# MasterVVK/qwen3-tts-axera-russian

Hardware: AMD Instinct MI355X
Metric: 12Hz codec-tokens/s (codec frames/s, 16 codes each) + RTF, Qwen3-TTS-0.6B (higher is better)
Workload: dtype f16 weights/KV, f32 accumulate (talker+CP); vocoder exact fp32 (f32 MFMA); 1 GPU; configs[2]/[3]: batch=32 mixed ru/en prompts per GPU, 64 frames/utterance/step (prefill + hipGraph decode loop), utterance-sharded DP over 1 GPU(s); batch_per_gpu=32

## Files before the change

include/qwen3tts_voc.h:

```cpp
#ifndef QWEN3TTS_VOC_H
#define QWEN3TTS_VOC_H

#include <stdint.h>

#ifdef __cplusplus
extern "C" {
#endif

#define Q3VOC_SAMPLES_PER_TOKEN 1920
#define Q3VOC_SAMPLE_RATE 24000

void* voc_load(const char* weights, int chunk_tokens, int max_batch);
void voc_free(void* v);
int voc_chunk_tokens(void* v);
int voc_samples_per_token(void* v);
int voc_chunk_samples(void* v);

int voc_decode(void* v, const int64_t* codes, int B, float* out);

int voc_synthesize(void* v, const int64_t* codes, int n_tokens, int16_t* out, int32_t* n_samples);
int voc_synthesize_f32(void* v, const int64_t* codes, int n_tokens, float* out, int32_t* n_samples);
int voc_synthesize_max_samples(void* v, int n_tokens);

int voc_synthesize_batch(void* v, const int64_t* codes, const int32_t* n_tokens, int U, int16_t* out, int64_t out_capacity,
// ... 16 lines not shown
int voc_stream_last_chunks(void* s);
float voc_stream_last_ms(void* s);

void* voc_incr_create(void* voc, int max_streams);
void voc_incr_free(void* s);
int voc_incr_reset(void* s, int stream);
int64_t voc_incr_push_max_samples(void* s, int n, const int32_t* streams, const int32_t* n_new, const int32_t* finish);
int voc_incr_push(void* s, int n, const int32_t* streams, const int64_t* codes, const int32_t* n_new, const int32_t* finish,
                  int16_t* out, int64_t out_capacity, int64_t* offsets);
int voc_incr_push_f32(void* s, int n, const int32_t* streams, const int64_t* codes, const int32_t* n_new, const int32_t* finish,
                      float* out, int64_t out_capacity, int64_t* offsets);
float voc_incr_last_ms(void* s);
int voc_incr_last_launches(void* s);
int64_t voc_incr_samples(void* voc, int64_t n_frames);
int64_t voc_incr_state_bytes(void* s);
int64_t voc_incr_device_bytes(void* s);

int voc_set_exact_fp32(int on);

int voc_set_fused_units(int on);

int voc_set_max_workgroups(int n);

float voc_last_decode_ms(void* v);
double voc_decode_flops(void* v, int B);

#ifdef __cplusplus
}
#endif
#endif
```

qwen3_tts_axera_russian_amd/csrc/q3_test_api.hip:

```cpp
#include "q3_model.h"
#include "q3_voc_ops.h"
#include <chrono>
#include <cstring>
#include <vector>

using namespace q3;

namespace q3 {
int set_linear_tuning(int K, int mt16, int kbw);
int set_linear_split_rows(int on);
int set_linear_narrow8(int on);
int set_linear_wide_tiles(int on);
int set_attn_short(int on);
int set_gemm_min_rows(int n);
int set_gemm_glds(int on);
int reset_linear_knobs();
const char* last_linear_variant();
}

namespace {
struct DBuf {
    void* p = nullptr;
    ~DBuf() {
        if (p) hipFree(p);
// ... 328 lines not shown
}

int q3t_voc_attn(int kernel, const float* x, float* y, int B, int H, int D, int L, int window, float theta) {
    constexpr float GUARD = 1234.5f;
    if ((kernel != 0 && kernel != 1) || !x || !y || B <= 0 || H <= 0 || D <= 0 || D > 128 || (D & 1) || L <= 0 || window <= 0)
        return -2;
    const int ld = (L + 31) / 32 * 32;
    const size_t nx = (size_t)B * 3 * H * D, ny = (size_t)B * H * D;
    std::vector<float> hx(nx * ld, 0.f), hy(ny * ld, GUARD);
    for (size_t r = 0; r < nx; r++) memcpy(hx.data() + r * ld, x + r * L, (size_t)L * 4);
    DBuf dx, dy;
    if (!dx.up(hx.data(), hx.size() * 4) || !dy.up(hy.data(), hy.size() * 4)) return -1;
    const int rc = kernel == 0 ? voc_launch_attn(nullptr, (const float*)dx.p, (float*)dy.p, H, D, L, ld, window, theta, B)
                               : voc_launch_attn_tile(nullptr, (const float*)dx.p, (float*)dy.p, H, D, L, ld, window, theta, B);
    if (rc) return -2;
    Q3_HIP(hipDeviceSynchronize(), -1);
    Q3_HIP(hipMemcpy(hy.data(), dy.p, hy.size() * 4, hipMemcpyDeviceToHost), -1);
    for (size_t r = 0; r < ny; r++) {
        memcpy(y + r * L, hy.data() + r * ld, (size_t)L * 4);
        for (int l = L; l < ld; l++)
            if (hy[r * ld + l] != GUARD) return -3;
    }
    return 0;
}

float q3t_bench_linear(int M, int N, int K, int pro, int epi, int nt, int n_copies, int iters) {
    hipStream_t s = nullptr;
    if (hipStreamCreate(&s) != hipSuccess) return -1.f;
    const size_t wbytes = (size_t)N * K * 2;
    const int Mreal = M;
    M = (M + 127) / 128 * 128;
    DBuf dW, dx, dh, dssq, dg, dy, dso, dact;
    if (!dW.alloc(wbytes * n_copies)) return -1.f;
    hipMemset(dW.p, 0x11, wbytes * n_copies);
    dx.alloc((size_t)M * K * 2);
    hipMemset(dx.p, 0, (size_t)M * K * 2);
    dh.alloc((size_t)M * K * 4);
    hipMemset(dh.p, 0, (size_t)M * K * 4);
    dssq.alloc((size_t)M * (K / 16) * 4);
    hipMemset(dssq.p, 0, (size_t)M * (K / 16) * 4);
    dg.alloc((size_t)K * 4);
    hipMemset(dg.p, 0, (size_t)K * 4);
    dy.alloc((size_t)M * N * 4);
    dso.alloc((size_t)M * (N / 16) * 4);
    dact.alloc((size_t)M * (N / 2) * 2);
    LinArgs a;
// ... 150 lines not shown
```

qwen3_tts_axera_russian_amd/csrc/q3_voc.hip:

```cpp
#include "../../include/qwen3tts_voc.h"
#include "q3_common.h"
#include "q3_voc_ops.h"

#include <algorithm>
#include <cmath>
#include <utility>

namespace q3 {

typedef float f16v __attribute__((ext_vector_type(16)));

enum { VOP_RVQ = 1, VOP_CONV = 2, VOP_CONVT = 3, VOP_DWCONV = 4, VOP_NORM = 5, VOP_ATTN = 6, VOP_GLU = 7, VOP_EMBMEAN = 8 };
enum { VF_SNAKE = 1, VF_RES_ADD = 2, VF_RES_SAVE = 4, VF_CLAMP = 8, VF_GELU = 16 };

__device__ __forceinline__ float gelu_erf(float x) { return 0.5f * x * (1.0f + erff(x * 0.70710678118654752f)); }
__device__ __forceinline__ float elu1(float x) { return x > 0.f ? x : expm1f(x); }


static int g_voc_split = 1;
static int g_voc_max_wgs = 0;
constexpr int VKC = 8;
constexpr int VTN = 128;
#ifndef Q3_VOC_XPAD
#define Q3_VOC_XPAD 1
#endif
#ifndef Q3_VOC_WPAD
#define Q3_VOC_WPAD 0
#endif
__host__ __device__ constexpr int voc_wpitch(int TM) { return Q3_VOC_WPAD ? (TM % 64 == 0 ? TM + 32 : (TM % 64 == 32 ? TM : TM + 4)) : TM + 4; }
__host__ __device__ inline int voc_xpitch(int XW) { return Q3_VOC_XPAD ? ((XW + 31) / 64) * 64 + 32 : XW; }

template <int MT, int KT, int KC, bool CT = false, int ACT = 3>
__global__ void __launch_bounds__(256, (KC >= 32 && MT >= 3) ? 2 : (MT >= 4 ? 3 : (MT == 3 ? 3 : 4))) conv_kernel(ConvArgs a) {
    constexpr int TM = 32 * MT, TMP = voc_wpitch(TM), Q = KC / 4;
    const int tid = threadIdx.x, lane = tid & 63, w = tid >> 6;
    const int halo = (KT - 1) * a.dil;
    const int HA = (halo + 3) & ~3;
    const int XW = VTN + HA;
    const int XP = voc_xpitch(XW);
    extern __shared__ __attribute__((aligned(16))) float lds[];
    float* Ws = lds;
    float* Xs = lds + KT * KC * TMP;
    for (int tile = blockIdx.x; tile < a.n_tiles; tile += gridDim.x) {
        const int lx = tile % a.tiles_l, my = (tile / a.tiles_l) % a.tiles_m, b = tile / (a.tiles_l * a.tiles_m);
        const int l0 = lx * VTN, m0 = my * TM;
        const float* xb = a.x + (size_t)b * a.Cin * a.ldx;
        const int Lcols = a.flat_B > 0 ? a.flat_B * a.ldx : a.Lc;
        f16v acc[MT];
#pragma unroll
        for (int mt = 0; mt < MT; mt++)
#pragma unroll
            for (int i = 0; i < 16; i++) acc[mt][i] = 0.f;
        constexpr int WN = KT * KC * (TM / 4), WIT = (WN + 255) / 256;
        constexpr int LPC = 256 / KC;
        constexpr int XJ1 = (VTN / 4 + LPC - 1) / LPC;
        const int xci = tid / LPC, xl = tid - xci * LPC;
        float4 wv[WIT];
        float4 xv1[KT == 1 ? XJ1 : 1];
        float al = 0.f, ib = 0.f;
        auto load_w = [&](int ci0) {
#pragma unroll
            for (int i = 0; i < WIT; i++) {
                const int idx = tid + i * 256, ic = idx < WN ? idx : 0;
                const int m4 = ic % (TM / 4), ci = (ic / (TM / 4)) % KC, k = ic / ((TM / 4) * KC);
                const int m = m0 + m4 * 4, mc = m < a.Mp ? m : 0, cg = ci0 + ci;
                wv[i] = *(const float4*)(a.wk + (unsigned)((((cg >> 3) * KT + k) * 8 + (cg & 7)) * a.Mp + mc));
// ... 146 lines not shown
                    }
                }
            }
        } else if (gl < Lcols) {
#pragma unroll
            for (int mt = 0; mt < MT; mt++)
#pragma unroll
                for (int r = 0; r < 16; r++) {
                    const int m = m0 + mt * 32 + (r & 3) + 8 * (r >> 2) + 4 * (lane >> 5);
                    if (m < a.M) {
                        const int co = a.stride == 1 ? m : m / a.stride;
                        const int p = a.stride == 1 ? 0 : m % a.stride;
                        const int jo = l * a.stride + p - a.lt;
                        if (a.stride != 1 && (jo < 0 || jo >= a.Lout)) continue;
                        const unsigned idx = (unsigned)((be * a.Cout + co) * a.ldy + jo);
                        float v = acc[mt][r];
                        if (a.bias) v += a.bias[co];
                        if (a.res) v += a.res[idx];
                        if (a.clamp) v = fminf(fmaxf(v, -1.f), 1.f);
                        __builtin_nontemporal_store(v, &a.y[idx]);
                    }
                }
        }
    }
}

template <int MT, int KT, int KC, bool CT = false, int ACT = -1>
static int launch_conv_t(hipStream_t s, const ConvArgs& a, int B) {
    if constexpr (!CT && KT <= 2) {
        if (a.stride > 1 && a.res == nullptr) return launch_conv_t<MT, KT, KC, true, ACT>(s, a, B);
    }
    if constexpr (ACT < 0) {
        if (a.elu) {
            if constexpr (!CT && KC == 16 && (KT == 1 || KT == 3)) return launch_conv_t<MT, KT, KC, CT, 4>(s, a, B);
            Q3_LOG("voc conv: ELU input is built for 1- and 3-tap convs at 16 channels per stage only");
            return -1;
        }
        if (a.alpha && a.gelu) {
            Q3_LOG("voc conv: Snake and GELU on one input are not built");
            return -1;
        }
        if constexpr (!(KT == 1 && KC == 16 && MT == 4 && !CT)) return launch_conv_t<MT, KT, KC, CT, 3>(s, a, B);
        else return a.alpha ? launch_conv_t<MT, KT, KC, CT, 1>(s, a, B) : a.gelu ? launch_conv_t<MT, KT, KC, CT, 2>(s, a, B)
                                                                             : launch_conv_t<MT, KT, KC, CT, 0>(s, a, B);
    } else {
    constexpr int TM = 32 * MT, TMP = voc_wpitch(TM);
    const int halo = (KT - 1) * a.dil;
// ... 8 lines not shown
        lds = lds_pad;
        static bool attr = false;
        if (!attr) {
            Q3_HIP(hipFuncSetAttribute((const void*)conv_kernel<MT, KT, KC, CT, ACT>, hipFuncAttributeMaxDynamicSharedMemorySize, 160 * 1024), -1);
            attr = true;
        }
    }
    ConvArgs c = a;
    c.Mp = (a.M + 3) / 4 * 4;
    c.flat_B = (KT == 1 && a.stride == 1) ? B : 0;
    if ((a.ldx & 3) || (a.ldy & 3) || a.ldx < a.Lin || a.ldy < a.Lout || a.Lc < a.Lin || a.Lc > a.Lin + KT - 1) {
        Q3_LOG("voc conv: bad geometry (Lin %d pitch %d, Lout %d pitch %d, Lc %d)", a.Lin, a.ldx, a.Lout, a.ldy, a.Lc);
        return -1;
    }
    {
        if ((size_t)B * a.Cin * a.ldx >= ((size_t)1 << 31) || (size_t)B * a.Cout * a.ldy >= ((size_t)1 << 31)) {
            Q3_LOG("voc conv: activation of %d x %d x %d / %d x %d x %d floats is beyond the kernel's 32-bit indexing", B, a.Cin, a.ldx, B, a.Cout, a.ldy);
            return -1;
        }
    }
    c.tiles_l = ((c.flat_B > 0 ? a.ldx * B : a.Lc) + VTN - 1) / VTN;
    c.tiles_m = (a.M + TM - 1) / TM;
    c.n_tiles = c.tiles_l * c.tiles_m * (c.flat_B > 0 ? 1 : B);
    int grid = c.n_tiles;
    if (g_voc_max_wgs > 0 && grid > g_voc_max_wgs) grid = g_voc_max_wgs;
    hipLaunchKernelGGL((conv_kernel<MT, KT, KC, CT, ACT>), dim3(grid), dim3(256), lds, s, c);
    Q3_HIP(hipGetLastError(), -1);
    return 0;
    }
}

template <int KT, int KC>
static int launch_conv_mt(hipStream_t s, const ConvArgs& a, int B) {
    const int t32 = (a.M + 31) / 32;
    int mt = 4;
    if (t32 % 4 != 0) mt = (t32 % 3 == 0) ? 3 : (t32 % 2 == 0) ? 2 : (t32 < 4 ? t32 : 4);
    static const int fill = getenv("Q3_VOC_FILL") ? atoi(getenv("Q3_VOC_FILL")) : 512;
    if (fill > 0) {
        const long cols = (KT == 1 && a.stride == 1) ? (long)a.ldx * B : (long)a.Lc;
        const long col_tiles = (cols + VTN - 1) / VTN * ((KT == 1 && a.stride == 1) ? 1 : B);
        while (mt > 1 && col_tiles * ((t32 + mt - 1) / mt) < fill) mt = (mt == 4 || mt == 2) ? mt / 2 : 1;
    }
    switch (mt) {
        case 1: return launch_conv_t<1, KT, KC>(s, a, B);
        case 2: return launch_conv_t<2, KT, KC>(s, a, B);
        case 3: return launch_conv_t<3, KT, KC>(s, a, B);
        default: return launch_conv_t<4, KT, KC>(s, a, B);
    }
// ... 77 lines not shown
        return a.K == 1 ? launch_conv_mt<1, 16>(s, a, B) : launch_conv_mt<2, 16>(s, a, B);
    switch (a.K) {
        case 1: return c % 32 == 0 ? launch_conv_mt<1, 32>(s, a, B) : c % 16 == 0 ? launch_conv_mt<1, 16>(s, a, B) : launch_conv_mt<1, 8>(s, a, B);
        case 2: return c % 32 == 0 ? launch_conv_mt<2, 32>(s, a, B) : c % 16 == 0 ? launch_conv_mt<2, 16>(s, a, B) : launch_conv_mt<2, 8>(s, a, B);
        case 3: return c % 16 == 0 ? launch_conv_mt<3, 16>(s, a, B) : launch_conv_mt<3, 8>(s, a, B);
        case 7: return launch_conv_mt<7, 8>(s, a, B);
        default:
            Q3_LOG("voc conv: kernel with %d taps is not built (1, 2, 3, 7 are)", a.K);
            return -1;
    }
}

int voc_launch_conv(hipStream_t s, const ConvArgs& a, int B) { return launch_conv(s, a, B); }

struct ResUnitArgs {
    const float* x = nullptr;
    float* y = nullptr;
    const float* w7 = nullptr;
    const float* w1p = nullptr;
    const float *b7 = nullptr, *b1 = nullptr;
    const float *al7 = nullptr, *ib7 = nullptr;
    const float *al1 = nullptr, *ib1 = nullptr;
    int Lin = 0, ld = 0, dil = 1, tiles_l = 0, n_tiles = 0;
};

static int g_voc_fuse = 1;

template <int MT>
__global__ void __launch_bounds__(256, MT <= 3 ? 3 : 2) resunit_kernel(ResUnitArgs a) {
    constexpr int C = 32 * MT, KT = 7, KC = 8, TMP = voc_wpitch(C);
    const int tid = threadIdx.x, lane = tid & 63, w = tid >> 6;
    const int halo = (KT - 1) * a.dil, HA = (halo + 3) & ~3, XW = VTN + HA, XP = voc_xpitch(XW);
    extern __shared__ __attribute__((aligned(16))) float lds[];
    float* Ws = lds;
    float* Xs = lds + KT * KC * TMP;
    float* Ps = Xs + KC * XP;
    for (int i = tid; i < C; i += 256) {
        Ps[i] = a.b7 ? a.b7[i] : 0.f;
        Ps[C + i] = a.al1[i];
        Ps[2 * C + i] = a.ib1[i];
        Ps[3 * C + i] = a.b1 ? a.b1[i] : 0.f;
    }
    for (int tile = blockIdx.x; tile < a.n_tiles; tile += gridDim.x) {
        const int lx = tile % a.tiles_l, b = tile / a.tiles_l;
        const int l0 = lx * VTN;
        const float* xb = a.x + (size_t)b * C * a.ld;
        f16v acc[MT];
#pragma unroll
        for (int mt = 0; mt < MT; mt++)
#pragma unroll
            for (int i = 0; i < 16; i++) acc[mt][i] = 0.f;
        for (int ci0 = 0; ci0 < C; ci0 += KC) {
            __syncthreads();
            constexpr int WN = KT * KC * (C / 4), WIT = (WN + 255) / 256;
            float4 wv[WIT];
#pragma unroll
            for (int i = 0; i < WIT; i++) {
                const int idx = tid + i * 256, ic = idx < WN ? idx : 0;
                const int m4 = ic % (C / 4), ci = (ic / (C / 4)) % KC, k = ic / ((C / 4) * KC);
                const int cg = ci0 + ci;
                wv[i] = *(const float4*)(a.w7 + (unsigned)((((cg >> 3) * KT + k) * 8 + (cg & 7)) * C + m4 * 4));
            }
            constexpr int LPC = 256 / KC, XG = (VTN + (((KT - 1) * 9 + 3) & ~3)) / 4, XJ = (XG + LPC - 1) / LPC;
            const int xci = tid / LPC, xl = tid - xci * LPC;
            const float al = a.al7[ci0 + xci], ib = a.ib7[ci0 + xci];
            float4 xv[XJ];
// ... 71 lines not shown
            for (int i = 0; i < MT; i++) {
                const int idx = tid + i * 256;
                *(float4*)(Ws + idx * 4) = *(const float4*)(a.w1p + (unsigned)(mt2 * 32 * C + idx * 4));
            }
            __syncthreads();
            f16v o;
#pragma unroll
            for (int i = 0; i < 16; i++) o[i] = 0.f;
#pragma unroll
            for (int mt = 0; mt < MT; mt++)
#pragma unroll
                for (int q = 0; q < 16; q++)
                    o = __builtin_amdgcn_mfma_f32_32x32x2f32(Ws[(mt * 16 + q) * 64 + lane], acc[mt][q], o, 0, 0, 0);
            if (live) {
                float* yb = a.y + (size_t)b * C * a.ld;
#pragma unroll
                for (int r = 0; r < 16; r++) {
                    const int mu = 32 * mt2 + (r & 3) + 8 * (r >> 2);
                    float* rowp = yb + (unsigned)(mu * a.ld);
                    __builtin_nontemporal_store(o[r] + Ps[3 * C + mu + 4 * (lane >> 5)] + res[r], &rowp[lane_off]);
                }
            }
        }
    }
}

template <int MT>
static int launch_resunit_t(hipStream_t s, ResUnitArgs a, int B) {
    constexpr int C = 32 * MT;
    const int halo = 6 * a.dil;
    if (a.dil > 9) return -1;
    const size_t lds = ((size_t)7 * 8 * voc_wpitch(C) + (size_t)8 * voc_xpitch(VTN + ((halo + 3) & ~3)) + 4 * C) * sizeof(float);
    a.tiles_l = (a.Lin + VTN - 1) / VTN;
    a.n_tiles = a.tiles_l * B;
    int grid = a.n_tiles;
    if (g_voc_max_wgs > 0 && grid > g_voc_max_wgs) grid = g_voc_max_wgs;
    hipLaunchKernelGGL((resunit_kernel<MT>), dim3(grid), dim3(256), lds, s, a);
    Q3_HIP(hipGetLastError(), -1);
    return 0;
}

static bool resunit_channels(int c) { return c == 96 || c == 192; }

static int launch_resunit(hipStream_t s, const ResUnitArgs& a, int C, int B) {
    return C == 96 ? launch_resunit_t<3>(s, a, B) : C == 192 ? launch_resunit_t<6>(s, a, B) : -1;
}

typedef _Float16 hv8 __attribute__((ext_vector_type(8)));

__global__ void __launch_bounds__(256) snake_split_kernel(const float* __restrict__ x, const float* __restrict__ alpha,
                                                          const float* __restrict__ inv_beta, _Float16* __restrict__ xh,
                                                          _Float16* __restrict__ xl, int C, int L, int ld, int gelu,
                                                          int* __restrict__ ovf) {
    const int l = blockIdx.x * 256 + threadIdx.x, cg = blockIdx.y, b = blockIdx.z;
    if (l >= L) return;
    const float* xp = x + ((size_t)b * C + cg * 8) * ld + l;
    float v[8];
#pragma unroll
    for (int j = 0; j < 8; j++) v[j] = xp[(size_t)j * ld];
// ... 20 lines not shown
    const size_t o = (((size_t)b * (C >> 3) + cg) * L + l) * 8;
    *(hv8*)(xh + o) = h;
    *(hv8*)(xl + o) = lo;
    if (big) *ovf = 1;
}

struct SplitArgs {
    const _Float16* xh = nullptr;
    const _Float16* xl = nullptr;
    float* y = nullptr;
    const _Float16* w_hi = nullptr;
    const _Float16* w_lo = nullptr;
    const float* bias = nullptr;
    const float* res = nullptr;
    _Float16* oh = nullptr;
    _Float16* ol = nullptr;
    const float* oalpha = nullptr;
    const float* oinv_beta = nullptr;
    int* ovf = nullptr;
    int Cin = 0, M = 0, Mp = 0, dil = 1, Lin = 0, stride = 1, Cout = 0, clamp = 0, B = 0;
    int ldy = 0, lt = 0, Lout = 0, Lc = 0;
    int n_tiles = 0, tiles_l = 0, tiles_m = 0;
    int my_fast = 0;
};

constexpr int SKC = 16;

template <int KT, int KS, int MW, int NJ>
__global__ void __launch_bounds__(256, NJ == 1 ? 3 : 2) conv_split_kernel(SplitArgs a) {
    constexpr int STM = 32 * MW, STN = 128 * NJ;
    constexpr int UNR = (MW == 3 && KT == 7) ? 1 : KS * KT;
    const int tid = threadIdx.x, lane = tid & 63, w = tid >> 6;
    const int halo = (KT - 1) * a.dil;
    const int XW = STN + halo;
    extern __shared__ __attribute__((aligned(16))) char slds[];
    _Float16* Wh = (_Float16*)slds;
    _Float16* Wl = Wh + KS * KT * STM * SKC;
    _Float16* Xh = Wl + KS * KT * STM * SKC;
    _Float16* Xl = Xh + (size_t)KS * XW * SKC;
    const int C16 = a.Cin >> 4;
    const hv8 zero8 = {0, 0, 0, 0, 0, 0, 0, 0};
    for (int tile = blockIdx.x; tile < a.n_tiles; tile += gridDim.x) {
        int lx, b, my;
        if (a.my_fast) {
            const int xcd = tile & 7, j = tile >> 3;
            my = j % a.tiles_m;
            const int cg = (j / a.tiles_m) * 8 + xcd;
            if (cg >= a.tiles_l * a.B) continue;
            lx = cg % a.tiles_l;
            b = cg / a.tiles_l;
        } else {
            lx = tile % a.tiles_l;
            b = (tile / a.tiles_l) % a.B;
            my = tile / (a.tiles_l * a.B);
        }
        const int l0 = lx * STN, m0 = my * STM;
        f16v acc[MW][NJ], accx[MW][NJ];
#pragma unroll
        for (int i = 0; i < MW; i++)
#pragma unroll
            for (int j = 0; j < NJ; j++)
#pragma unroll
                for (int r = 0; r < 16; r++) {
                    acc[i][j][r] = 0.f;
                    accx[i][j][r] = 0.f;
// ... 86 lines not shown
                        if (a.oh && mg < a.M) {
                            hv4 vh, vl;
                            bool big = false;
#pragma unroll
                            for (int q = 0; q < 4; q++) {
                                float t = v[q];
                                if (a.oalpha) {
                                    const float sn = __sinf(a.oalpha[mg + q] * t);
                                    t = t + a.oinv_beta[mg + q] * (sn * sn);
                                }
                                big |= !(fabsf(t) <= 65504.f);
                                const _Float16 hi = (_Float16)fminf(fmaxf(t, -65504.f), 65504.f);
                                vh[q] = hi;
                                vl[q] = (_Float16)((t - (float)hi) * 2048.0f);
                            }
                            if (big) *a.ovf = 1;
                            const size_t o = (((size_t)b * (a.Cout >> 3) + (mg >> 3)) * a.Lin + l) * 8 + (mg & 7);
                            *(hv4*)(a.oh + o) = vh;
                            *(hv4*)(a.ol + o) = vl;
                        }
                    }
                }
            }
    }
}

template <int KT, int KS, int MW, int NJ>
static int launch_conv_split_t(hipStream_t s, const SplitArgs& a, int B) {
    constexpr int STM = 32 * MW, STN = 128 * NJ;
    if (a.dil > 9) return -1;
    const int halo = (KT - 1) * a.dil;
    const size_t lds = ((size_t)2 * KS * KT * STM * SKC + (size_t)2 * KS * (STN + halo) * SKC) * sizeof(_Float16);
    static bool set_ = false;
    if (!set_) {
        Q3_HIP(hipFuncSetAttribute((const void*)conv_split_kernel<KT, KS, MW, NJ>, hipFuncAttributeMaxDynamicSharedMemorySize, 80 * 1024), -1);
        set_ = true;
    }
    if (lds > 80 * 1024 || (a.Cin / 16) % KS || a.Mp % STM) return -1;
    SplitArgs c = a;
    c.B = B;
    c.tiles_l = (a.Lc + STN - 1) / STN;
    c.tiles_m = (a.M + STM - 1) / STM;
    c.n_tiles = c.tiles_l * c.tiles_m * B;
    c.my_fast = c.tiles_m > 1 && (size_t)a.Cin * a.Mp * KT * 4 <= (size_t)2 << 20;
    if (c.my_fast) c.n_tiles = (c.tiles_l * B + 7) / 8 * 8 * c.tiles_m;
    int grid = c.n_tiles;
    if (g_voc_max_wgs > 0 && grid > g_voc_max_wgs) grid = g_voc_max_wgs;
    hipLaunchKernelGGL((conv_split_kernel<KT, KS, MW, NJ>), dim3(grid), dim3(256), lds, s, c);
    Q3_HIP(hipGetLastError(), -1);
    return 0;
}

static int g_voc_narrow_k1 = 1;

template <int MW>
static int launch_conv_split_m(hipStream_t s, const SplitArgs& a, int K, int B) {
    const int c16 = a.Cin / 16;
    switch (K) {
        case 1:
            if (g_voc_narrow_k1 && MW == 3)
                return c16 % 3 == 0 ? launch_conv_split_t<1, 3, MW, 1>(s, a, B) : c16 % 2 == 0 ? launch_conv_split_t<1, 2, MW, 1>(s, a, B) : launch_conv_split_t<1, 1, MW, 1>(s, a, B);
            return c16 % 3 == 0 ? launch_conv_split_t<1, 3, MW, 2>(s, a, B) : c16 % 2 == 0 ? launch_conv_split_t<1, 2, MW, 2>(s, a, B) : launch_conv_split_t<1, 1, MW, 2>(s, a, B);
        case 2:
            if (g_voc_narrow_k1 && MW == 3 && a.Cin <= 384)
                return c16 % 2 == 0 ? launch_conv_split_t<2, 2, MW, 1>(s, a, B) : launch_conv_split_t<2, 1, MW, 1>(s, a, B);
            return c16 % 2 == 0 ? launch_conv_split_t<2, 2, MW, 2>(s, a, B) : launch_conv_split_t<2, 1, MW, 2>(s, a, B);
        case 3: return c16 % 2 == 0 && MW == 2 ? launch_conv_split_t<3, 2, MW, 2>(s, a, B) : launch_conv_split_t<3, 1, MW, 2>(s, a, B);
        case 7:
            if (g_voc_narrow_k1 && a.Cin <= 192) return launch_conv_split_t<7, 1, MW, 1>(s, a, B);
            return launch_conv_split_t<7, 1, MW, 2>(s, a, B);
// ... 426 lines not shown

struct Voc {
    int device = 0;
    int chunk = 64, max_batch = 1, upsample = 1;
    long chunk_samples = 0;
    std::vector<VocOp> ops;
    std::vector<void*> allocs;
    hipStream_t s = nullptr;
    hipEvent_t e0 = nullptr, e1 = nullptr;
    int64_t* d_codes = nullptr;
    int* d_ovf = nullptr;
    bool warned_ovf = false;
    float *buf[3] = {nullptr, nullptr, nullptr};
    _Float16 *plane[4] = {nullptr, nullptr, nullptr, nullptr};
    size_t buf_elems = 0;
    float last_ms = 0.f;
    double flops_per_chunk = 0.0;
    float* d_wave = nullptr;
    int16_t* d_wave16 = nullptr;
    size_t wave_cap = 0, wave16_cap = 0;
    ChunkPlace* d_place = nullptr;
    float batch_ms = 0.f;
    int batch_chunks = 0;
};

static float* voc_up(Voc* v, const PackTensor* t) {
    size_t ne = t->numel();
    std::vector<float> tmp;
    const float* src = (const float*)t->data;
    if (t->dtype == F16) {
        tmp.resize(ne);
        for (size_t i = 0; i < ne; i++) tmp[i] = h2f(((const uint16_t*)t->data)[i]);
        src = tmp.data();
    } else if (t->dtype != F32) {
        return nullptr;
    }
    float* d = nullptr;
    if (hipMalloc((void**)&d, ne * 4) != hipSuccess) return nullptr;
    v->allocs.push_back(d);
    if (hipMemcpy(d, src, ne * 4, hipMemcpyHostToDevice) != hipSuccess) return nullptr;
    return d;
}

static float* voc_up_host(Voc* v, const std::vector<float>& h) {
    float* d = nullptr;
    if (hipMalloc((void**)&d, h.size() * 4) != hipSuccess) return nullptr;
    v->allocs.push_back(d);
    if (hipMemcpy(d, h.data(), h.size() * 4, hipMemcpyHostToDevice) != hipSuccess) return nullptr;
    return d;
}

static void voc_destroy(Voc* v) {
    if (!v) return;
    if (v->s) hipStreamSynchronize(v->s);
    for (void* p : v->allocs) hipFree(p);
    for (float* b : v->buf)
        if (b) hipFree(b);
    for (_Float16* b : v->plane)
        if (b) hipFree(b);
    if (v->d_codes) hipFree(v->d_codes);
    if (v->d_wave) hipFree(v->d_wave);
    if (v->d_wave16) hipFree(v->d_wave16);
    if (v->d_place) hipFree(v->d_place);
    if (v->d_ovf) hipFree(v->d_ovf);
    if (v->e0) hipEventDestroy(v->e0);
    if (v->e1) hipEventDestroy(v->e1);
    if (v->s) hipStreamDestroy(v->s);
    delete v;
}

}

using namespace q3;

static inline void voc_bind(const Voc* v) {
    int d = -1;
    if (v && (hipGetDevice(&d) != hipSuccess || d != v->device)) hipSetDevice(v->device);
}

extern "C" {

void voc_free(void* vv) {
    voc_bind((Voc*)vv);
    voc_destroy((Voc*)vv);
}

void* voc_load(const char* weights, int chunk_tokens, int max_batch) {
// ... 314 lines not shown
        Q3_LOG("voc_load failed");
        voc_destroy(v);
        return nullptr;
    }
    return v;
}

int voc_set_exact_fp32(int on) {
    g_voc_split = on ? 0 : 1;
    return 0;
}

int voc_set_narrow_k1(int on) {
    g_voc_narrow_k1 = on ? 1 : 0;
    return 0;
}

int voc_set_fused_units(int on) {
    g_voc_fuse = on ? 1 : 0;
    return 0;
}

int voc_set_max_workgroups(int n) {
    if (n < 0) {
        int dev = 0;
        hipDeviceProp_t p;
        n = (hipGetDevice(&dev) == hipSuccess && hipGetDeviceProperties(&p, dev) == hipSuccess) ? p.multiProcessorCount : 0;
    }
    g_voc_max_wgs = n;
    return n;
}

int voc_chunk_tokens(void* vv) { return vv ? ((Voc*)vv)->chunk : 0; }
int voc_samples_per_token(void* vv) { return vv ? ((Voc*)vv)->upsample : 0; }
int voc_chunk_samples(void* vv) { return vv ? (int)((Voc*)vv)->chunk_samples : 0; }
float voc_last_decode_ms(void* vv) { return vv ? ((Voc*)vv)->last_ms : -1.f; }
double voc_decode_flops(void* vv, int B) { return vv ? ((Voc*)vv)->flops_per_chunk * B : 0.0; }

struct SplitState {
    int f32_idx = 0;
    bool f32_cur = true;
    int planes = -1;
    float* res = nullptr;
};

static bool split_capable(const VocOp& op) { return (op.op == VOP_CONV || op.op == VOP_CONVT) && op.w_hi != nullptr; }

static int voc_conv_split(Voc* v, const VocOp& op, const VocOp* next, bool last, int B, int C, long L, SplitState& st) {
    const int KT = op.op == VOP_CONV ? op.k : op.k / op.p0;
    int in_set = st.planes;
    if (in_set < 0) {
        if (!st.f32_cur) return -1;
        in_set = 0;
// ... 40 lines not shown
        out_f32 = st.f32_idx ^ 1;
        if (sa.res == v->buf[out_f32]) return -1;
        sa.y = v->buf[out_f32];
    }
    if (want_planes) {
        sa.oh = v->plane[2 * (in_set ^ 1)];
        sa.ol = v->plane[2 * (in_set ^ 1) + 1];
        if (next->flags & VF_SNAKE) {
            sa.oalpha = next->alpha;
            sa.oinv_beta = next->inv_beta;
        }
    }
    if (launch_conv_split(v->s, sa, KT, B)) return -1;
    if (want_f32) {
        st.f32_idx = out_f32;
        st.f32_cur = true;
    } else {
        st.f32_cur = false;
    }
    st.planes = want_planes ? (in_set ^ 1) : -1;
    return 0;
}

static int voc_run(Voc* v, int B, float** out_dev, int n_ops = -1, int* outC = nullptr, long* outL = nullptr,
                   float* op_ms = nullptr, bool force_exact = false, int T = 0) {
    int cur = 0;
    int C = 0;
    if (T <= 0 || T > v->chunk) T = v->chunk;
    long L = T;
    long Lf = v->chunk;
    float* res = nullptr;
    SplitState st;
    const size_t nrun = n_ops < 0 ? v->ops.size() : (size_t)n_ops < v->ops.size() ? (size_t)n_ops : v->ops.size();
    for (size_t i = 0; i < nrun; i++) {
        const VocOp& op = v->ops[i];
        if (op_ms) hipEventRecord(v->e0, v->s);
        float* in = v->buf[cur];
        float* out = v->buf[cur ^ 1];
        const int ld = (int)pitch4(L);
        if (op.op == VOP_RVQ || op.op == VOP_EMBMEAN) {
            if (op.op == VOP_RVQ)
                hipLaunchKernelGGL(rvq_kernel, dim3(T, B), dim3(256), 2 * op.cin * sizeof(float), v->s, v->d_codes, op.w,
                                   op.p_sem, op.p_ac, out, T, ld, op.nq, op.cb, op.cin, op.cout);
            else
                hipLaunchKernelGGL(embmean_kernel, dim3(T, B), dim3(256), 0, v->s, v->d_codes, op.w, out, T, ld,
                                   op.nq, 16, op.cb, op.cout);
            Q3_HIP(hipGetLastError(), -1);
            C = op.cout;
// ... 1125 lines not shown
```

qwen3_tts_axera_russian_amd/csrc/q3_voc_ops.h:

```cpp
#pragma once
#include <hip/hip_runtime.h>

namespace q3 {

struct ConvArgs {
    const float* x = nullptr;
    float* y = nullptr;
    const float* wk = nullptr;
    int Mp = 0;
    const float* bias = nullptr;
    const float* alpha = nullptr;
    const float* inv_beta = nullptr;
    const float* res = nullptr;
    int gelu = 0;
    int Cin = 0, M = 0, K = 0, dil = 1, Lin = 0, stride = 1, Cout = 0, clamp = 0;
    int ldx = 0, ldy = 0;
    int lt = 0, Lout = 0, Lc = 0;
    int Lrule = 0;
    int n_tiles = 0, tiles_l = 0, tiles_m = 0;
    int flat_B = 0;
    int elu = 0;
};

int voc_launch_conv(hipStream_t s, const ConvArgs& a, int B);
int voc_launch_norm(hipStream_t s, const float* x, const float* w, const float* bias, float* y, int C, int L, int ld,
                    int kind, float eps, int B);
int voc_launch_attn(hipStream_t s, const float* x, float* y, int H, int D, int L, int ld, int window, float theta, int B);
int voc_launch_attn_tile(hipStream_t s, const float* x, float* y, int H, int D, int L, int ld, int window, float theta, int B);

}
```

qwen3_tts_axera_russian_amd/hiplib.py:

```python
from __future__ import annotations

import ctypes
import os

from . import LIB_PATH, TEST_LIB_PATH

_lib = None
_test_lib = None

c_void_p, c_int, c_float, c_char_p = ctypes.c_void_p, ctypes.c_int, ctypes.c_float, ctypes.c_char_p
f32p = ctypes.POINTER(ctypes.c_float)
i32p = ctypes.POINTER(ctypes.c_int32)
i64p = ctypes.POINTER(ctypes.c_int64)
u16p = ctypes.POINTER(ctypes.c_uint16)
i16p = ctypes.POINTER(ctypes.c_int16)


class SlotParamsC(ctypes.Structure):
    _fields_ = [("max_frames", ctypes.c_int32), ("temperature", ctypes.c_float), ("top_k", ctypes.c_int32),
                ("top_p", ctypes.c_float), ("cp_temperature", ctypes.c_float), ("cp_top_k", ctypes.c_int32),
                ("seed", ctypes.c_uint64), ("utt", ctypes.c_int32), ("reserved", ctypes.c_int32)]


def _sig(lib, name, restype, argtypes):
# ... 44 lines not shown
    _sig(lib, "q3e_set_forced_codes", c_int, [c_void_p, i32p, c_int])
    _sig(lib, "q3e_start", c_int, [c_void_p, c_int, f32p, i32p, i32p, c_int, c_int])
    _sig(lib, "q3e_run", c_int, [c_void_p, c_int])
    _sig(lib, "q3e_last_run_ms", c_float, [c_void_p])
    _sig(lib, "q3e_last_prefill_ms", c_float, [c_void_p])
    _sig(lib, "q3e_get_codes", c_int, [c_void_p, i32p, c_int, i32p])
    _sig(lib, "q3e_get_done", c_int, [c_void_p, i32p, i32p])
    _sig(lib, "q3e_refill", c_int, [c_void_p, c_int, i32p, f32p, i32p, i32p])
    _sig(lib, "q3e_open", c_int, [c_void_p, c_int, c_int])
    _sig(lib, "q3e_admit", c_int, [c_void_p, c_int, i32p, f32p, i32p, i32p, ctypes.POINTER(SlotParamsC)])
    _sig(lib, "q3e_release", c_int, [c_void_p, c_int, i32p])
    _sig(lib, "q3e_get_hidden", c_int, [c_void_p, f32p])
    _sig(lib, "q3e_step_weight_bytes", ctypes.c_double, [c_void_p])
    _sig(lib, "voc_load", c_void_p, [c_char_p, c_int, c_int])
    _sig(lib, "voc_free", None, [c_void_p])
    _sig(lib, "voc_chunk_tokens", c_int, [c_void_p])
    _sig(lib, "voc_samples_per_token", c_int, [c_void_p])
    _sig(lib, "voc_chunk_samples", c_int, [c_void_p])
    _sig(lib, "voc_decode", c_int, [c_void_p, i64p, c_int, f32p])
    _sig(lib, "voc_synthesize", c_int, [c_void_p, i64p, c_int, i16p, i32p])
    _sig(lib, "voc_synthesize_f32", c_int, [c_void_p, i64p, c_int, f32p, i32p])
    _sig(lib, "voc_synthesize_max_samples", c_int, [c_void_p, c_int])
    _sig(lib, "voc_set_max_workgroups", c_int, [c_int])
    _sig(lib, "voc_set_exact_fp32", c_int, [c_int])
    _sig(lib, "voc_set_fused_units", c_int, [c_int])
    _sig(lib, "voc_last_decode_ms", c_float, [c_void_p])
    _sig(lib, "voc_decode_flops", ctypes.c_double, [c_void_p, c_int])
    i64p_ = ctypes.POINTER(ctypes.c_int64)
    _sig(lib, "voc_synthesize_batch", c_int, [c_void_p, i64p, i32p, c_int, i16p, ctypes.c_int64, i64p_])
    _sig(lib, "voc_synthesize_batch_f32", c_int, [c_void_p, i64p, i32p, c_int, f32p, ctypes.c_int64, i64p_])
    _sig(lib, "voc_synthesize_batch_max_samples", ctypes.c_int64, [c_void_p, i32p, c_int])
    _sig(lib, "voc_last_batch_ms", c_float, [c_void_p])
    _sig(lib, "voc_last_batch_chunks", c_int, [c_void_p])
    _sig(lib, "voc_stream_create", c_void_p, [c_void_p, c_int])
    _sig(lib, "voc_stream_free", None, [c_void_p])
    _sig(lib, "voc_stream_reset", c_int, [c_void_p, c_int])
    _sig(lib, "voc_stream_push_max_samples", ctypes.c_int64, [c_void_p, c_int, i32p, i32p, i32p])
    _sig(lib, "voc_stream_push", c_int, [c_void_p, c_int, i32p, i64p, i32p, i32p, i16p, ctypes.c_int64, i64p_])
    _sig(lib, "voc_stream_push_f32", c_int, [c_void_p, c_int, i32p, i64p, i32p, i32p, f32p, ctypes.c_int64, i64p_])
    _sig(lib, "voc_stream_last_decodes", c_int, [c_void_p])
    _sig(lib, "voc_stream_last_chunks", c_int, [c_void_p])
    _sig(lib, "voc_stream_last_ms", c_float, [c_void_p])
    _sig(lib, "voc_incr_create", c_void_p, [c_void_p, c_int])
    _sig(lib, "voc_incr_free", None, [c_void_p])
    _sig(lib, "voc_incr_reset", c_int, [c_void_p, c_int])
    _sig(lib, "voc_incr_push_max_samples", ctypes.c_int64, [c_void_p, c_int, i32p, i32p, i32p])
# ... 37 lines not shown
    if not os.path.exists(TEST_LIB_PATH):
        raise RuntimeError(f"{TEST_LIB_PATH} not found: build it with `python -m qwen3_tts_axera_russian_amd.build`")
    lib = ctypes.CDLL(TEST_LIB_PATH)
    _sig(lib, "q3t_set_linear_tuning", c_int, [c_int, c_int, c_int])
    _sig(lib, "q3t_linear", c_int, [c_int, c_int, c_int, u16p, c_int, c_int, c_int, u16p, f32p, f32p, c_float,
                                    f32p, f32p, u16p, c_int])
    _sig(lib, "q3t_linear_case", c_int, [c_int, c_int, c_int, c_int, u16p, c_int, c_int, c_int, c_int, c_float, c_int,
                                         u16p, f32p, f32p, f32p, f32p, f32p, u16p, f32p, f32p, f32p, u16p, u16p])
    _sig(lib, "q3t_reset_linear_knobs", c_int, [])
    _sig(lib, "q3t_last_linear_variant", c_char_p, [])
    _sig(lib, "q3t_talker_sample", c_int, [f32p, c_int, i32p, c_int, c_int, c_int])
    _sig(lib, "q3t_attn", c_int, [c_int, c_int, c_int, f32p, f32p, f32p, c_float, f32p, f32p, c_int, i32p, i32p, c_int,
                                  c_int, c_int, c_int, u16p, u16p, c_int, c_int, i32p, c_int, c_int, c_int, c_int, u16p])
    _sig(lib, "q3t_voc_attn", c_int, [c_int, f32p, f32p, c_int, c_int, c_int, c_int, c_int, c_float])
    _sig(lib, "q3t_set_linear_split_rows", c_int, [c_int])
    _sig(lib, "q3t_set_linear_narrow8", c_int, [c_int])
    _sig(lib, "q3t_set_linear_wide_tiles", c_int, [c_int])
    _sig(lib, "q3t_set_attn_short", c_int, [c_int])
    _sig(lib, "q3t_set_gemm_min_rows", c_int, [c_int])
    _sig(lib, "q3t_set_gemm_glds", c_int, [c_int])
    _sig(lib, "q3t_inspect_weights", c_int, [ctypes.c_char_p, ctypes.c_char_p, ctypes.c_char_p, c_int])
    _sig(lib, "q3t_bench_linear", c_float, [c_int, c_int, c_int, c_int, c_int, c_int, c_int, c_int])
    _sig(lib, "q3t_bench_chain", c_float, [c_int, c_int, c_int, c_int, c_int, c_int])
    _test_lib = lib
    return lib


def fptr(a):
    return a.ctypes.data_as(f32p)


def iptr(a):
    return a.ctypes.data_as(i32p)
```

Measured before the change: 8941 codec_frames/s.

## Confine vocoder conv tiles to a CU subset via atomic work-claiming

```diff
diff --git a/include/qwen3tts_voc.h b/include/qwen3tts_voc.h
--- a/include/qwen3tts_voc.h
+++ b/include/qwen3tts_voc.h
@@ -62,6 +62,8 @@
 
 int voc_set_max_workgroups(int n);
 
+int voc_set_corun_cus(int k);
+
 float voc_last_decode_ms(void* v);
 double voc_decode_flops(void* v, int B);
 
diff --git a/qwen3_tts_axera_russian_amd/csrc/q3_test_api.hip b/qwen3_tts_axera_russian_amd/csrc/q3_test_api.hip
--- a/qwen3_tts_axera_russian_amd/csrc/q3_test_api.hip
+++ b/qwen3_tts_axera_russian_amd/csrc/q3_test_api.hip
@@ -374,6 +374,69 @@
             if (hy[r * ld + l] != GUARD) return -3;
     }
     return 0;
+}
+
+namespace {
+__global__ void __launch_bounds__(256) cu_key_probe_kernel(unsigned* seen) {
+    if (threadIdx.x == 0) atomicAdd(seen + voc_cu_key(), 1u);
+    for (int i = 0; i < 200; i++) __builtin_amdgcn_s_sleep(16);
+}
+}
+
+int q3t_cu_key_probe(int blocks, unsigned* keys, int cap) {
+    if (blocks <= 0 || blocks > (1 << 16) || !keys || cap < VP_KEYS) return -2;
+    DBuf d;
+    if (!d.alloc(sizeof(unsigned) * VP_KEYS)) return -1;
+    Q3_HIP(hipMemset(d.p, 0, sizeof(unsigned) * VP_KEYS), -1);
+    hipLaunchKernelGGL(cu_key_probe_kernel, dim3(blocks), dim3(256), 0, nullptr, (unsigned*)d.p);
+    Q3_HIP(hipGetLastError(), -1);
+    Q3_HIP(hipDeviceSynchronize(), -1);
+    Q3_HIP(hipMemcpy(keys, d.p, sizeof(unsigned) * VP_KEYS, hipMemcpyDeviceToHost), -1);
+    int n = 0;
+    for (int i = 0; i < VP_KEYS; i++) n += keys[i] != 0;
+    return n;
+}
+
+int q3t_voc_part_stat_arm(int words) { return (words > 0) == (voc_part_stat(words) != nullptr) ? 0 : -1; }
+int q3t_voc_part_stat_read(unsigned* out, int words) {
+    unsigned* d = voc_part_stat(-1);
+    if (!d || !out || words <= 0) return -2;
+    Q3_HIP(hipDeviceSynchronize(), -1);
+    Q3_HIP(hipMemcpy(out, d, sizeof(unsigned) * words, hipMemcpyDeviceToHost), -1);
+    Q3_HIP(hipMemset(d, 0, sizeof(unsigned) * words), -1);
+    return 0;
+}
+
+int q3t_voc_part_conv(int C, int L, int B, unsigned* visits, int cap, unsigned* units) {
+    if (C <= 0 || C % 8 || L <= 0 || B <= 0 || !visits || !units || cap <= 0) return -2;
+    const int ld = (L + 31) / 32 * 32;
+    DBuf dx, dy, dw;
+    const size_t na = (size_t)B * C * ld * 4, nw = (size_t)C * 7 * ((C + 3) / 4 * 4) * 4;
+    if (!dx.alloc(na) || !dy.alloc(na) || !dw.alloc(nw)) return -1;
+    Q3_HIP(hipMemset(dx.p, 0, na), -1);
+    Q3_HIP(hipMemset(dw.p, 0, nw), -1);
+    if (!voc_part_stat(VP_KEYS + cap)) return -1;
+    ConvArgs a;
+    a.x = (const float*)dx.p;
+    a.y = (float*)dy.p;
+    a.wk = (const float*)dw.p;
+    a.Cin = a.Cout = a.M = C;
+    a.K = 7;
+    a.Lin = a.Lout = a.Lc = L;
+    a.ldx = a.ldy = ld;
+    VocPartRun run;
+    int rc = voc_part_begin(&run, nullptr);
+    if (!rc) rc = voc_launch_conv(nullptr, a, B);
+    const int tiles = voc_last_launch_tiles();
+    voc_part_end();
+    if (!rc) rc = hipDeviceSynchronize() == hipSuccess ? 0 : -1;
+    if (!rc && tiles > cap) rc = -3;
+    if (!rc) rc = hipMemcpy(units, voc_part_stat(-1), sizeof(unsigned) * VP_KEYS, hipMemcpyDeviceToHost) == hipSuccess ? 0 : -1;
+    if (!rc && tiles > 0)
+        rc = hipMemcpy(visits, voc_part_stat(-1) + VP_KEYS, sizeof(unsigned) * tiles, hipMemcpyDeviceToHost) == hipSuccess ? 0 : -1;
+    voc_part_release(&run);
+    voc_part_stat(0);
+    return rc ? rc : tiles;
 }
 
 float q3t_bench_linear(int M, int N, int K, int pro, int epi, int nt, int n_copies, int iters) {
diff --git a/qwen3_tts_axera_russian_amd/csrc/q3_voc.hip b/qwen3_tts_axera_russian_amd/csrc/q3_voc.hip
--- a/qwen3_tts_axera_russian_amd/csrc/q3_voc.hip
+++ b/qwen3_tts_axera_russian_amd/csrc/q3_voc.hip
@@ -4,6 +4,7 @@
 
 #include <algorithm>
 #include <cmath>
+#include <mutex>
 #include <utility>
 
 namespace q3 {
@@ -19,6 +20,154 @@
 
 static int g_voc_split = 1;
 static int g_voc_max_wgs = 0;
+
+__host__ __device__ constexpr int conv_residency(int MT, int KC) { return (KC >= 32 && MT >= 3) ? 2 : (MT >= 4 ? 3 : (MT == 3 ? 3 : 4)); }
+__host__ __device__ constexpr int resunit_residency(int MT) { return MT <= 3 ? 3 : 2; }
+__host__ __device__ constexpr int split_residency(int NJ) { return NJ == 1 ? 3 : 2; }
+
+__device__ __forceinline__ int voc_part_enter(const VocPart& p, int* sh) {
+    if (threadIdx.x == 0) {
+        const unsigned key = voc_cu_key();
+        int* st = p.cus + key;
+        int s = __hip_atomic_load(st, __ATOMIC_RELAXED, __HIP_MEMORY_SCOPE_AGENT);
+        if (s == 0) {
+            s = atomicCAS(st, 0, 3);
+            if (s == 0) {
+                s = atomicAdd(p.cus + 2 * VP_KEYS + (key >> 8), 1) < p.per_xcd ? 1 : 2;
+                atomicExch(st, s);
+            }
+        }
+        int work = 0;
+        if (s == 1) {
+            if (atomicAdd(p.cus + VP_KEYS + key, 1) < p.slots) work = 1;
+            else atomicSub(p.cus + VP_KEYS + key, 1);
+        }
+        if (!work && atomicAdd(p.ctr + 1, 1u) == gridDim.x - 1) work = 2;
+        sh[1] = work;
+    }
+    __syncthreads();
+    return sh[1];
+}
+__device__ __forceinline__ int voc_part_claim(const VocPart& p, int* sh) {
+    __syncthreads();
+    if (threadIdx.x == 0) {
+        const unsigned t = atomicAdd(p.ctr, 1u);
+        sh[0] = t < 0x7fffffffu ? (int)t : 0x7fffffff;
+    }
+    __syncthreads();
+    return sh[0];
+}
+__device__ __forceinline__ void voc_part_leave(const VocPart& p, int work) {
+    if (threadIdx.x == 0 && work == 1) {
+        atomicSub(p.cus + VP_KEYS + voc_cu_key(), 1);
+        atomicAdd(p.ctr + 1, 1u);
+    }
+}
+__device__ __forceinline__ void voc_part_count(const VocPart& p, int tile) {
+    if (p.stat && threadIdx.x == 0) {
+        atomicAdd(p.stat + voc_cu_key(), 1u);
+        if (tile < p.stat_tiles) atomicAdd(p.stat + VP_KEYS + tile, 1u);
+    }
+}
+#define VOC_TILE_WALK_BEGIN(a)                                                     \
+    __shared__ int vp_sh[2];                                                       \
+    const bool vp_claim = (a).part.ctr != nullptr;                                 \
+    int vp_work = 0;                                                               \
+    if (vp_claim) {                                                                \
+        vp_work = voc_part_enter((a).part, vp_sh);                                 \
+        if (!vp_work) return;                                                      \
+    }                                                                              \
+    for (int tile = vp_claim ? voc_part_claim((a).part, vp_sh) : (int)blockIdx.x; tile < (a).n_tiles; \
+         tile = vp_claim ? voc_part_claim((a).part, vp_sh) : tile + (int)gridDim.x) {                 \
+        if (vp_claim) voc_part_count((a).part, tile);
+#define VOC_TILE_WALK_END(a) \
+    }                        \
+    if (vp_claim) voc_part_leave((a).part, vp_work);
+
+constexpr int VP_RING = 1024;
+constexpr int VP_MAX_DEV = 16;
+constexpr int VP_DEFAULT_CUS = 128;
+static bool g_voc_corun = false;
+static int g_corun_k = getenv("Q3_VOC_CORUN_CUS") ? atoi(getenv("Q3_VOC_CORUN_CUS")) / 8 * 8 : VP_DEFAULT_CUS;
+static const int g_corun_slots = getenv("Q3_VOC_CORUN_SLOTS") ? atoi(getenv("Q3_VOC_CORUN_SLOTS")) : 0;
+static const int g_corun_grid = getenv("Q3_VOC_CORUN_GRID") ? atoi(getenv("Q3_VOC_CORUN_GRID")) : 1;
+static int* g_part_cus[VP_MAX_DEV] = {};
+static int g_part_ncu[VP_MAX_DEV] = {};
+static unsigned* g_part_stat = nullptr;
+static int g_part_stat_tiles = 0;
+static thread_local VocPartRun* t_part = nullptr;
+static thread_local hipStream_t t_part_stream = nullptr;
+static thread_local int t_last_tiles = 0;
+
+static int voc_part_table(int* dev_out) {
+    static std::mutex mu;
+    std::lock_guard<std::mutex> lock(mu);
+    int dev = 0;
+    if (hipGetDevice(&dev) != hipSuccess || dev < 0 || dev >= VP_MAX_DEV) return -1;
+    if (!g_part_cus[dev]) {
+        const size_t bytes = sizeof(int) * (2 * VP_KEYS + 16);
+        hipDeviceProp_t p;
+        if (hipGetDeviceProperties(&p, dev) != hipSuccess) return -1;
+        if (hipMalloc((void**)&g_part_cus[dev], bytes) != hipSuccess || hipMemset(g_part_cus[dev], 0, bytes) != hipSuccess) return -1;
+        g_part_ncu[dev] = p.multiProcessorCount;
+    }
+    *dev_out = dev;
+    return 0;
+}
+
+int voc_part_begin(VocPartRun* r, hipStream_t s) {
+    t_part = nullptr;
+    if (!g_voc_corun || g_corun_k <= 0) return 0;
+    int dev = 0;
+    if (voc_part_table(&dev)) return -1;
+    if (!r->ring) Q3_HIP(hipMalloc((void**)&r->ring, sizeof(unsigned) * 2 * VP_RING), -1);
+    Q3_HIP(hipMemsetAsync(r->ring, 0, sizeof(unsigned) * 2 * VP_RING, s), -1);
+    r->pos = 0;
+    t_part = r;
+    t_part_stream = s;
+    return 0;
+}
+void voc_part_end() { t_part = nullptr; }
+void voc_part_release(VocPartRun* r) {
+    if (r->ring) hipFree(r->ring);
+    r->ring = nullptr;
+}
+int voc_last_launch_tiles() { return t_last_tiles; }
+unsigned* voc_part_stat(int words) {
+    if (words < 0) return g_part_stat;
+    if (g_part_stat) {
+        hipDeviceSynchronize();
+        hipFree(g_part_stat);
+        g_part_stat = nullptr;
+    }
+    g_part_stat_tiles = words > VP_KEYS ? words - VP_KEYS : 0;
+    if (words > 0 && words < VP_KEYS) return nullptr;
+    if (words > 0 && (hipMalloc((void**)&g_part_stat, sizeof(unsigned) * words) != hipSuccess ||
+                      hipMemset(g_part_stat, 0, sizeof(unsigned) * words) != hipSuccess))
+        g_part_stat = nullptr;
+    return g_part_stat;
+}
+
+static int voc_walk(int n_tiles, int residency, hipStream_t s, VocPart* part) {
+    int grid = n_tiles;
+    if (g_voc_max_wgs > 0 && grid > g_voc_max_wgs) grid = g_voc_max_wgs;
+    t_last_tiles = 0;
+    VocPartRun* r = t_part;
+    int dev = 0;
+    if (!r || s != t_part_stream || !g_voc_corun || g_corun_k <= 0 || r->pos >= VP_RING || voc_part_table(&dev)) return grid;
+    const int k = g_corun_k < g_part_ncu[dev] ? g_corun_k : g_part_ncu[dev] / 8 * 8;
+    const int slots = residency + g_corun_slots > 1 ? residency + g_corun_slots : 1;
+    if (k < 8 || (long)n_tiles <= (long)slots * k) return grid;
+    part->ctr = r->ring + 2 * r->pos++;
+    part->cus = g_part_cus[dev];
+    part->per_xcd = k / 8;
+    part->slots = slots;
+    part->stat = g_part_stat;
+    part->stat_tiles = g_part_stat_tiles;
+    t_last_tiles = n_tiles;
+    const long full = (long)residency * g_part_ncu[dev] * (g_corun_grid > 1 ? g_corun_grid : 1);
+    return (int)(n_tiles < full ? n_tiles : full);
+}
 constexpr int VKC = 8;
 constexpr int VTN = 128;
 #ifndef Q3_VOC_XPAD
@@ -31,7 +180,7 @@
 __host__ __device__ inline int voc_xpitch(int XW) { return Q3_VOC_XPAD ? ((XW + 31) / 64) * 64 + 32 : XW; }
 
 template <int MT, int KT, int KC, bool CT = false, int ACT = 3>
-__global__ void __launch_bounds__(256, (KC >= 32 && MT >= 3) ? 2 : (MT >= 4 ? 3 : (MT == 3 ? 3 : 4))) conv_kernel(ConvArgs a) {
+__global__ void __launch_bounds__(256, conv_residency(MT, KC)) conv_kernel(ConvArgs a) {
     constexpr int TM = 32 * MT, TMP = voc_wpitch(TM), Q = KC / 4;
     const int tid = threadIdx.x, lane = tid & 63, w = tid >> 6;
     const int halo = (KT - 1) * a.dil;
@@ -41,7 +190,7 @@
     extern __shared__ __attribute__((aligned(16))) float lds[];
     float* Ws = lds;
     float* Xs = lds + KT * KC * TMP;
-    for (int tile = blockIdx.x; tile < a.n_tiles; tile += gridDim.x) {
+    VOC_TILE_WALK_BEGIN(a)
         const int lx = tile % a.tiles_l, my = (tile / a.tiles_l) % a.tiles_m, b = tile / (a.tiles_l * a.tiles_m);
         const int l0 = lx * VTN, m0 = my * TM;
         const float* xb = a.x + (size_t)b * a.Cin * a.ldx;
@@ -234,7 +383,7 @@
                     }
                 }
         }
-    }
+    VOC_TILE_WALK_END(a)
 }
 
 template <int MT, int KT, int KC, bool CT = false, int ACT = -1>
@@ -289,8 +438,7 @@
     c.tiles_l = ((c.flat_B > 0 ? a.ldx * B : a.Lc) + VTN - 1) / VTN;
     c.tiles_m = (a.M + TM - 1) / TM;
     c.n_tiles = c.tiles_l * c.tiles_m * (c.flat_B > 0 ? 1 : B);
-    int grid = c.n_tiles;
-    if (g_voc_max_wgs > 0 && grid > g_voc_max_wgs) grid = g_voc_max_wgs;
+    const int grid = voc_walk(c.n_tiles, conv_residency(MT, KC), s, &c.part);
     hipLaunchKernelGGL((conv_kernel<MT, KT, KC, CT, ACT>), dim3(grid), dim3(256), lds, s, c);
     Q3_HIP(hipGetLastError(), -1);
     return 0;
@@ -414,12 +562,13 @@
     const float *al7 = nullptr, *ib7 = nullptr;
     const float *al1 = nullptr, *ib1 = nullptr;
     int Lin = 0, ld = 0, dil = 1, tiles_l = 0, n_tiles = 0;
+    VocPart part;
 };
 
 static int g_voc_fuse = 1;
 
 template <int MT>
-__global__ void __launch_bounds__(256, MT <= 3 ? 3 : 2) resunit_kernel(ResUnitArgs a) {
+__global__ void __launch_bounds__(256, resunit_residency(MT)) resunit_kernel(ResUnitArgs a) {
     constexpr int C = 32 * MT, KT = 7, KC = 8, TMP = voc_wpitch(C);
     const int tid = threadIdx.x, lane = tid & 63, w = tid >> 6;
     const int halo = (KT - 1) * a.dil, HA = (halo + 3) & ~3, XW = VTN + HA, XP = voc_xpitch(XW);
@@ -433,7 +582,7 @@
         Ps[2 * C + i] = a.ib1[i];
         Ps[3 * C + i] = a.b1 ? a.b1[i] : 0.f;
     }
-    for (int tile = blockIdx.x; tile < a.n_tiles; tile += gridDim.x) {
+    VOC_TILE_WALK_BEGIN(a)
         const int lx = tile % a.tiles_l, b = tile / a.tiles_l;
         const int l0 = lx * VTN;
         const float* xb = a.x + (size_t)b * C * a.ld;
@@ -551,7 +700,7 @@
                 }
             }
         }
-    }
+    VOC_TILE_WALK_END(a)
 }
 
 template <int MT>
@@ -562,8 +711,7 @@
     const size_t lds = ((size_t)7 * 8 * voc_wpitch(C) + (size_t)8 * voc_xpitch(VTN + ((halo + 3) & ~3)) + 4 * C) * sizeof(float);
     a.tiles_l = (a.Lin + VTN - 1) / VTN;
     a.n_tiles = a.tiles_l * B;
-    int grid = a.n_tiles;
-    if (g_voc_max_wgs > 0 && grid > g_voc_max_wgs) grid = g_voc_max_wgs;
+    const int grid = voc_walk(a.n_tiles, resunit_residency(MT), s, &a.part);
     hipLaunchKernelGGL((resunit_kernel<MT>), dim3(grid), dim3(256), lds, s, a);
     Q3_HIP(hipGetLastError(), -1);
     return 0;
@@ -630,12 +778,13 @@
     int ldy = 0, lt = 0, Lout = 0, Lc = 0;
     int n_tiles = 0, tiles_l = 0, tiles_m = 0;
     int my_fast = 0;
+    VocPart part;
 };
 
 constexpr int SKC = 16;
 
 template <int KT, int KS, int MW, int NJ>
-__global__ void __launch_bounds__(256, NJ == 1 ? 3 : 2) conv_split_kernel(SplitArgs a) {
+__global__ void __launch_bounds__(256, split_residency(NJ)) conv_split_kernel(SplitArgs a) {
     constexpr int STM = 32 * MW, STN = 128 * NJ;
     constexpr int UNR = (MW == 3 && KT == 7) ? 1 : KS * KT;
     const int tid = threadIdx.x, lane = tid & 63, w = tid >> 6;
@@ -648,7 +797,7 @@
     _Float16* Xl = Xh + (size_t)KS * XW * SKC;
     const int C16 = a.Cin >> 4;
     const hv8 zero8 = {0, 0, 0, 0, 0, 0, 0, 0};
-    for (int tile = blockIdx.x; tile < a.n_tiles; tile += gridDim.x) {
+    VOC_TILE_WALK_BEGIN(a)
         int lx, b, my;
         if (a.my_fast) {
             const int xcd = tile & 7, j = tile >> 3;
@@ -781,7 +930,7 @@
                     }
                 }
             }
-    }
+    VOC_TILE_WALK_END(a)
 }
 
 template <int KT, int KS, int MW, int NJ>
@@ -803,8 +952,7 @@
     c.n_tiles = c.tiles_l * c.tiles_m * B;
     c.my_fast = c.tiles_m > 1 && (size_t)a.Cin * a.Mp * KT * 4 <= (size_t)2 << 20;
     if (c.my_fast) c.n_tiles = (c.tiles_l * B + 7) / 8 * 8 * c.tiles_m;
-    int grid = c.n_tiles;
-    if (g_voc_max_wgs > 0 && grid > g_voc_max_wgs) grid = g_voc_max_wgs;
+    const int grid = voc_walk(c.n_tiles, split_residency(NJ), s, &c.part);
     hipLaunchKernelGGL((conv_split_kernel<KT, KS, MW, NJ>), dim3(grid), dim3(256), lds, s, c);
     Q3_HIP(hipGetLastError(), -1);
     return 0;
@@ -1277,6 +1425,7 @@
     ChunkPlace* d_place = nullptr;
     float batch_ms = 0.f;
     int batch_chunks = 0;
+    VocPartRun part;
 };
 
 static float* voc_up(Voc* v, const PackTensor* t) {
@@ -1318,6 +1467,7 @@
     if (v->d_wave16) hipFree(v->d_wave16);
     if (v->d_place) hipFree(v->d_place);
     if (v->d_ovf) hipFree(v->d_ovf);
+    voc_part_release(&v->part);
     if (v->e0) hipEventDestroy(v->e0);
     if (v->e1) hipEventDestroy(v->e1);
     if (v->s) hipStreamDestroy(v->s);
@@ -1678,13 +1828,33 @@
 }
 
 int voc_set_max_workgroups(int n) {
-    if (n < 0) {
-        int dev = 0;
-        hipDeviceProp_t p;
-        n = (hipGetDevice(&dev) == hipSuccess && hipGetDeviceProperties(&p, dev) == hipSuccess) ? p.multiProcessorCount : 0;
-    }
+    int dev = 0;
+    hipDeviceProp_t p;
+    const int cus = (hipGetDevice(&dev) == hipSuccess && hipGetDeviceProperties(&p, dev) == hipSuccess) ? p.multiProcessorCount : 0;
+    if (n < 0) n = cus;
+    g_voc_corun = n > 0 && n == cus;
     g_voc_max_wgs = n;
     return n;
+}
+
+int voc_set_corun_cus(int k) {
+    int dev = 0, ncu = 0;
+    hipDeviceProp_t p;
+    if (hipGetDevice(&dev) == hipSuccess && hipGetDeviceProperties(&p, dev) == hipSuccess) ncu = p.multiProcessorCount;
+    if (k < 0) k = VP_DEFAULT_CUS;
+    k = k / 8 * 8;
+    if (ncu > 0 && k > ncu / 8 * 8) k = ncu / 8 * 8;
+    if (k != g_corun_k) {
+        for (int d = 0; d < VP_MAX_DEV; d++)
+            if (g_part_cus[d]) {
+                hipSetDevice(d);
+                hipDeviceSynchronize();
+                hipMemset(g_part_cus[d], 0, sizeof(int) * (2 * VP_KEYS + 16));
+            }
+        hipSetDevice(dev);
+    }
+    g_corun_k = k;
+    return k;
 }
 
 int voc_chunk_tokens(void* vv) { return vv ? ((Voc*)vv)->chunk : 0; }
@@ -1771,8 +1941,15 @@
     return 0;
 }
 
+static int voc_run_ops(Voc* v, int B, float** out_dev, int n_ops, int* outC, long* outL, float* op_ms, bool force_exact, int T);
 static int voc_run(Voc* v, int B, float** out_dev, int n_ops = -1, int* outC = nullptr, long* outL = nullptr,
                    float* op_ms = nullptr, bool force_exact = false, int T = 0) {
+    if (voc_part_begin(&v->part, v->s)) return -1;
+    const int rc = voc_run_ops(v, B, out_dev, n_ops, outC, outL, op_ms, force_exact, T);
+    voc_part_end();
+    return rc;
+}
+static int voc_run_ops(Voc* v, int B, float** out_dev, int n_ops, int* outC, long* outL, float* op_ms, bool force_exact, int T) {
     int cur = 0;
     int C = 0;
     if (T <= 0 || T > v->chunk) T = v->chunk;
diff --git a/qwen3_tts_axera_russian_amd/csrc/q3_voc_ops.h b/qwen3_tts_axera_russian_amd/csrc/q3_voc_ops.h
--- a/qwen3_tts_axera_russian_amd/csrc/q3_voc_ops.h
+++ b/qwen3_tts_axera_russian_amd/csrc/q3_voc_ops.h
@@ -2,6 +2,25 @@
 #include <hip/hip_runtime.h>
 
 namespace q3 {
+
+constexpr int VP_KEYS = 16 * 256;
+struct VocPart {
+    unsigned* ctr = nullptr;
+    int* cus = nullptr;
+    int per_xcd = 0;
+    int slots = 0;
+    unsigned* stat = nullptr;
+    int stat_tiles = 0;
+};
+
+#ifdef __HIPCC__
+__device__ __forceinline__ unsigned voc_cu_key() {
+    unsigned xcc, hw;
+    asm volatile("s_getreg_b32 %0, hwreg(HW_REG_XCC_ID)" : "=s"(xcc));
+    asm volatile("s_getreg_b32 %0, hwreg(HW_REG_HW_ID)" : "=s"(hw));
+    return ((xcc & 15u) << 8) | ((hw >> 8) & 255u);
+}
+#endif
 
 struct ConvArgs {
     const float* x = nullptr;
@@ -20,7 +39,18 @@
     int n_tiles = 0, tiles_l = 0, tiles_m = 0;
     int flat_B = 0;
     int elu = 0;
+    VocPart part;
 };
+
+struct VocPartRun {
+    unsigned* ring = nullptr;
+    int pos = 0;
+};
+int voc_part_begin(VocPartRun* r, hipStream_t s);
+void voc_part_end();
+void voc_part_release(VocPartRun* r);
+int voc_last_launch_tiles();
+unsigned* voc_part_stat(int words);
 
 int voc_launch_conv(hipStream_t s, const ConvArgs& a, int B);
 int voc_launch_norm(hipStream_t s, const float* x, const float* w, const float* bias, float* y, int C, int L, int ld,
diff --git a/qwen3_tts_axera_russian_amd/hiplib.py b/qwen3_tts_axera_russian_amd/hiplib.py
--- a/qwen3_tts_axera_russian_amd/hiplib.py
+++ b/qwen3_tts_axera_russian_amd/hiplib.py
@@ -90,6 +90,7 @@
     _sig(lib, "voc_synthesize_f32", c_int, [c_void_p, i64p, c_int, f32p, i32p])
     _sig(lib, "voc_synthesize_max_samples", c_int, [c_void_p, c_int])
     _sig(lib, "voc_set_max_workgroups", c_int, [c_int])
+    _sig(lib, "voc_set_corun_cus", c_int, [c_int])
     _sig(lib, "voc_set_exact_fp32", c_int, [c_int])
     _sig(lib, "voc_set_fused_units", c_int, [c_int])
     _sig(lib, "voc_last_decode_ms", c_float, [c_void_p])
@@ -173,6 +174,11 @@
     _sig(lib, "q3t_inspect_weights", c_int, [ctypes.c_char_p, ctypes.c_char_p, ctypes.c_char_p, c_int])
     _sig(lib, "q3t_bench_linear", c_float, [c_int, c_int, c_int, c_int, c_int, c_int, c_int, c_int])
     _sig(lib, "q3t_bench_chain", c_float, [c_int, c_int, c_int, c_int, c_int, c_int])
+    u32p = ctypes.POINTER(ctypes.c_uint32)
+    _sig(lib, "q3t_cu_key_probe", c_int, [c_int, u32p, c_int])
+    _sig(lib, "q3t_voc_part_stat_arm", c_int, [c_int])
+    _sig(lib, "q3t_voc_part_stat_read", c_int, [u32p, c_int])
+    _sig(lib, "q3t_voc_part_conv", c_int, [c_int, c_int, c_int, u32p, c_int, u32p])
     _test_lib = lib
     return lib
 
```

Result: slower. 6590 codec_frames/s (-26.3%).
